# AleoNet/snarkVM

Hardware: AMD Instinct MI355X
Metric: BLS12-377 G1 MSM scalar-point pairs/sec (+ Fr NTT elements/sec in ntt_*) (higher is better)
Workload: dtype u32 limbs (29-bit radix) modular integer arithmetic, Fq 377-bit / Fr 253-bit; 1 GPU; G1 Pippenger MSM 2^24 (BASELINE.json configs[1]), bases (i+1)G registered in HBM, uniform scalars in HBM; independent instance per GPU; scalars=uniform, lg_ntt=24, window_bits=auto, base_tables=12, table_bits=22, pipelined_batch=True

## Files before the change

### snarkvm_amd/csrc/msm.hip.h

```cpp
#pragma once
#include <stdlib.h>

#include <type_traits>

#include "ec.hip.h"
#include "ffl.hip.h"
#include "ffl2.hip.h"
#include "hex2.hip.h"
#include "tuning.hip.h"

namespace sv {

struct msm_plan_t {
    size_t n;
    int c;
    int W;
    int J;
    int Wd;
    uint32_t nb;
    uint32_t nbt;
    uint32_t chunk;
    uint32_t nchunks;
    uint32_t S, S2;
    uint32_t L;
    int rounds;
    uint32_t bias[10];
};

static inline int msm_pick_c(size_t n) {
    if (n > ((size_t)1 << 17)) return 16;
    int lg = 0;
    while (((size_t)1 << lg) < n) lg++;
    int c = lg - 4;
    if (c < 2) c = 2;
    if (c > 11) c = 11;
    return c;
}
static constexpr int MSM_C_MAX = 23;
static constexpr int MSM_BIAS_BITS = 288;
static inline msm_plan_t msm_make_plan(size_t n, int c_override = 0, int tables = 1, int table_bits = 0) {
    msm_plan_t p;
    p.n = n;
    p.J = tables < 1 ? 1 : tables;
    if (p.J == 1) {
        p.c = c_override ? c_override : msm_pick_c(n);
        if (p.c > 16) p.c = 16;
        p.W = (254 + p.c - 1) / p.c;
    } else {
        const int part = table_bits > 0 ? table_bits : 256 / p.J;
        if (c_override) {
            p.c = c_override;
            if (p.c > part) p.c = part;
            while (part % p.c) p.c--;
            if (p.c > 16 && p.c != part) {
                p.c = 16;
                while (part % p.c) p.c--;
            }
            if (p.c < 2) p.c = part <= 16 ? part : 2;
        } else if (part <= 16) {
            p.c = n >= 4096 ? 16 : 8;
            if (p.c > part) p.c = part;
            while (part % p.c) p.c--;
            if (p.c < 2) p.c = part;
        } else {
            double best = 0;
            p.c = 0;
            for (int d = 2; d <= part && d <= MSM_C_MAX; d++) {
                if (part % d || (d > 16 && d != part)) continue;
                const double cost = (double)p.J * (part / d) * (double)n + (double)(part / d) * (double)((size_t)1 << (d - 1)) * 8.0;
                if (p.c == 0 || cost < best) {
                    best = cost;
                    p.c = d;
                }
            }
            if (p.c == 0) p.c = 1;
        }
        p.W = part / p.c;
    }
    p.Wd = p.W * p.J;
    p.nb = 1u << (p.c - 1);
    p.nbt = (uint32_t)p.W * p.nb;
    p.chunk = (1u << 18) / (uint32_t)p.J;
    p.chunk &= ~7u;
    if (p.chunk > n) p.chunk = (uint32_t)(n ? n : 1);
    p.nchunks = (uint32_t)((n + p.chunk - 1) / p.chunk);
    const int env_S = tuning().seg, env_S2 = tuning().seg2, env_L = tuning().fold_l;
    {
        const size_t E = (size_t)p.Wd * n;
        const size_t smax = E >= ((size_t)1 << 27) ? 128 : 64, round = (size_t)1 << 16;
        const size_t k = (E + smax * round - 1) / (smax * round);
        const size_t sfill = k ? (E + k * round - 1) / (k * round) : 4;
        p.S = (uint32_t)(sfill < 4 ? 4 : sfill);
    }
    if (env_S > 0) p.S = env_S;
    p.S2 = env_S2 > 1 ? env_S2 : 16;
    p.L = env_L > 0 ? (uint32_t)env_L : 8;
    if (p.L > p.nb) p.L = p.nb;
    while (p.nb % p.L) p.L--;
    p.rounds = 0;
    size_t m = ((size_t)p.J * n + p.S - 1) / p.S;
    while (m > 1) {
        m = (m + p.S2 - 1) / p.S2;
        p.rounds++;
    }
    for (int i = 0; i < 10; i++) p.bias[i] = 0;
    for (int w = 0; w < p.Wd; w++) {
        int bit = p.c - 1 + p.c * w;
        if (bit >= MSM_BIAS_BITS) break;
        p.bias[bit / 32] |= 1u << (bit % 32);
    }
    return p;
}

static constexpr int SCAN_TILE = 2048;
static __global__ void scan_tile_kernel(const uint32_t* in, uint32_t* out, uint32_t* block_sums, size_t n) {
    __shared__ uint32_t sh[256];
    const size_t base = (size_t)blockIdx.x * SCAN_TILE + (size_t)threadIdx.x * 8;
    uint32_t v[8], s = 0;
#pragma unroll
    for (int i = 0; i < 8; i++) {
        v[i] = (base + i < n) ? in[base + i] : 0u;
        s += v[i];
    }
    sh[threadIdx.x] = s;
    __syncthreads();
    for (int off = 1; off < 256; off <<= 1) {
        uint32_t t = (threadIdx.x >= (unsigned)off) ? sh[threadIdx.x - off] : 0u;
        __syncthreads();
        sh[threadIdx.x] += t;
        __syncthreads();
    }
    uint32_t run = sh[threadIdx.x] - s;
#pragma unroll
    for (int i = 0; i < 8; i++) {
        if (base + i < n) out[base + i] = run;
        run += v[i];
    }
    if (threadIdx.x == 255 && block_sums) block_sums[blockIdx.x] = sh[255];
}
static __global__ void scan_add_kernel(uint32_t* out, const uint32_t* block_offsets, size_t n) {
    const size_t base = (size_t)blockIdx.x * SCAN_TILE + (size_t)threadIdx.x * 8;
    const uint32_t add = block_offsets[blockIdx.x];
#pragma unroll
    for (int i = 0; i < 8; i++)
        if (base + i < n) out[base + i] += add;
}
static inline size_t scan_tmp_elems(size_t n) {
// ... 765 lines not shown
```

### snarkvm_amd/csrc/msm_sort.hip.h

```cpp
#pragma once
#include "ffl.hip.h"
#include "ffl2.hip.h"
#include "ffl2p.hip.h"
#include "msm.hip.h"

namespace sv {

static constexpr int SORT_TILE = 8192;
static constexpr int SORT_THREADS = 256;

struct msm_inst_t {
    const uint4* scalars;
    uint32_t n;
    uint32_t n0;
    uint32_t off0, off1;
    uint32_t pstart;
    uint32_t ptiles;
};
struct msm_radix_params_t {
    size_t n;
    int c, W, J;
    int HB, LB;
    uint32_t nb;
    uint32_t tiles_per_row;
    uint32_t TPW;
    const msm_inst_t* inst = nullptr;
    uint32_t ninst = 0;
    uint32_t vstride = 0, vn0 = 0, vr0 = 0, vr1 = 0;
    uint32_t xcd = 0;
};
__device__ __forceinline__ uint32_t xcd_tile(uint32_t b, uint32_t T) {
    const uint32_t q = T >> 3, r = T & 7u, x = b & 7u;
    return (x < r ? x * (q + 1) : r * (q + 1) + (x - r) * q) + (b >> 3);
}
struct l1_tile_t {
    uint32_t w, tw, TPW, j;
    size_t cbase;
    size_t row;
    size_t lo, hi;
    uint32_t inst_idx;
};
__device__ __forceinline__ l1_tile_t l1_decode_tile(const msm_radix_params_t& p, uint32_t g) {
    l1_tile_t t;
    const uint32_t B1 = 1u << p.HB;
    if (!p.inst) {
        t.w = g / p.TPW;
        t.tw = g - t.w * p.TPW;
        t.TPW = p.TPW;
        t.j = t.tw / p.tiles_per_row;
        const uint32_t tt = t.tw - t.j * p.tiles_per_row;
        t.cbase = (size_t)t.w * B1 * p.TPW;
        t.row = (size_t)(t.j * p.W + t.w) * p.n;
        t.lo = (size_t)tt * SORT_TILE;
        t.hi = (t.lo + SORT_TILE < p.n) ? t.lo + SORT_TILE : p.n;
        t.inst_idx = 0;
        return t;
    }
// ... 690 lines not shown
__global__ void __launch_bounds__(256, 1) msm_accumulate_lazy_kernel(const g1_aff_mem_t* __restrict__ bases, const uint32_t* __restrict__ sorted,
                                                              const uint32_t* __restrict__ boff, const uint32_t* __restrict__ start,
                                                              g1_lazy_partial_t* __restrict__ partial, uint32_t nbt, uint32_t S, uint32_t debug_idx_mask) {
    const uint32_t t = blockIdx.x * blockDim.x + threadIdx.x;
    const uint32_t total = boff[nbt];
    const uint64_t lo64 = (uint64_t)t * S;
    if (lo64 >= total) return;
    const uint32_t lo = (uint32_t)lo64;
    const uint32_t hi = (total - lo < S) ? total : lo + S;
    uint32_t k = find_bucket(boff, nbt, lo);
    uint32_t kend = boff[k + 1];
    uint32_t kend2 = boff[k + 2 <= nbt ? k + 2 : nbt];
    uint32_t start_k = start[k];
    uint32_t part_off = t - boff[k] / S;
    xyzz_lazy_t acc = xyzz_lazy_t::infinity();
    auto slot_of = [&](uint32_t e) -> const g1_lazy_slot_t* { return (const g1_lazy_slot_t*)&bases[(e & 0x7fffffffu) & debug_idx_mask]; };
    uint32_t e_cur = sorted[lo];
    uint32_t e_n1 = lo + 1 < hi ? sorted[lo + 1] : 0u;
    g1_lazy_slot_t raw_next = *slot_of(e_cur);
    for (uint32_t pos = lo;; pos++) {
        const bool end = pos >= hi;
        if (end || pos >= kend) {
            acc.store_raw(&partial[start_k + part_off]);
            if (end) break;
            part_off = 0;
            acc.inf = true;
            k++;
            kend = kend2;
            while (pos >= kend) {
                k++;
                kend = boff[k + 1];
            }
            kend2 = boff[k + 2 <= nbt ? k + 2 : nbt];
            start_k = start[k];
        }
        const uint32_t e = e_cur;
        const g1_lazy_slot_t raw = raw_next;
        if (pos + 1 < hi) raw_next = *slot_of(e_n1);
        e_cur = e_n1;
        if (pos + 2 < hi) e_n1 = sorted[pos + 2];
        if (raw.w[26]) continue;
        const bool neg = (e >> 31) != 0;
        fql_t px, py;
        raw.coords(px, py);
        if (!acc.madd(px, py, neg)) {
            xyzz_lazy_t tmp = acc;
            const fql_t tx = px, ty = py;
            lazy_exceptional_add(&tmp, &tx, &ty, neg);
            acc = tmp;
        }
    }
}

static __global__ void __launch_bounds__(256) g2_pair_partials_to_exact_kernel(const g2_pair_partial_t* __restrict__ raw, xyzz_mem_t<fq2_t>* __restrict__ partial,
                                                                        const uint32_t* __restrict__ start, uint32_t nbt) {
    const uint32_t g = blockIdx.x * blockDim.x + threadIdx.x;
    const uint32_t i = g >> 3, k = g & 7;
    if (i >= start[nbt]) return;
    const uint4* q = (const uint4*)&raw[i].w[16 * k];
    uint32_t t[16];
#pragma unroll
    for (int j = 0; j < 4; j++) {
        const uint4 u = q[j];
        t[4 * j] = u.x, t[4 * j + 1] = u.y, t[4 * j + 2] = u.z, t[4 * j + 3] = u.w;
    }
    fql_t c;
#pragma unroll
    for (int j = 0; j < 13; j++) c.v[j] = (int32_t)t[j];
    c.to_exact().store(&((fq_mem_t*)&partial[i])[k]);
}
template <bool PREFETCH>
__global__ void __launch_bounds__(256, 2) msm_accumulate_pair2_kernel(const aff_mem_t<fq2_t>* __restrict__ bases, const uint32_t* __restrict__ sorted,
                                                               const uint32_t* __restrict__ boff, const uint32_t* __restrict__ start,
                                                               g2_pair_partial_t* __restrict__ partial, uint32_t nbt, uint32_t S, uint32_t debug_idx_mask) {
    const uint32_t gt = blockIdx.x * blockDim.x + threadIdx.x;
    const uint32_t t = gt >> 1;
    const int comp = (int)(gt & 1u);
    const uint32_t total = boff[nbt];
    const uint64_t lo64 = (uint64_t)t * S;
    if (lo64 >= total) return;
    const uint32_t lo = (uint32_t)lo64;
    const uint32_t hi = (total - lo < S) ? total : lo + S;
    uint32_t k = find_bucket(boff, nbt, lo);
    uint32_t kend = boff[k + 1];
    uint32_t start_k = start[k];
    uint32_t part_off = t - boff[k] / S;
    fq2p::xyzz_pair_t<fq2p::xp_dev> acc;
    acc.inf = true;
    auto slot_of = [&](uint32_t e) -> const g2_lazy_slot_t* { return (const g2_lazy_slot_t*)&bases[(e & 0x7fffffffu) & debug_idx_mask]; };
    for (uint32_t pos = lo;; pos++) {
        const bool end = pos >= hi;
        if (end || pos >= kend) {
            uint4* q = (uint4*)&partial[start_k + part_off].w[16 * comp];
            if (acc.inf) {
#pragma unroll
                for (int c4 = 0; c4 < 4; c4++)
#pragma unroll
                    for (int j = 0; j < 4; j++) q[8 * c4 + j] = make_uint4(0, 0, 0, 0);
            } else {
                const fql_t* cs[4] = {&acc.x[0], &acc.y[0], &acc.zz[0], &acc.zzz[0]};
#pragma unroll
                for (int c4 = 0; c4 < 4; c4++) {
                    const int32_t* v = cs[c4]->v;
                    q[8 * c4 + 0] = make_uint4((uint32_t)v[0], (uint32_t)v[1], (uint32_t)v[2], (uint32_t)v[3]);
                    q[8 * c4 + 1] = make_uint4((uint32_t)v[4], (uint32_t)v[5], (uint32_t)v[6], (uint32_t)v[7]);
                    q[8 * c4 + 2] = make_uint4((uint32_t)v[8], (uint32_t)v[9], (uint32_t)v[10], (uint32_t)v[11]);
// ... 23 lines not shown
```

### snarkvm_amd/csrc/runtime.hip.h

```cpp
#pragma once
#include <hip/hip_runtime.h>
#include <stdint.h>
#include <stdio.h>
#include <stdlib.h>
#include <string.h>
#include <time.h>

#include <atomic>
#include <chrono>
#include <condition_variable>
#include <deque>
#include <functional>
#include <exception>
#include <memory>
#include <mutex>
#include <stdexcept>
#include <string>
#include <thread>
#include <type_traits>
#include <utility>
#include <vector>

#include "../../include/snarkvm_hip.h"
#include "ec.hip.h"
// ... 53 lines not shown
        size_t want = bytes + bytes / 8 + 256;
        alloc_timer_t timer(0, want);
        if (p) sv_defer_free(p);
        p = nullptr;
        cap = 0;
        if (hipMalloc(&p, want) != hipSuccess) {
            (void)hipGetLastError();
            p = nullptr;
            sv_drain_frees();
            const hipError_t e = hipMalloc(&p, want);
            if (e != hipSuccess) {
                (void)hipGetLastError();
                p = nullptr;
                throw hip_failure{e, "hipMalloc", __LINE__};
            }
        }
        cap = want;
    }
    template <class T>
    T* as() const {
        return (T*)p;
    }
};
struct pinned_buf {
    void* p = nullptr;
    size_t cap = 0;
    void ensure(size_t bytes) {
        if (bytes <= cap) return;
        size_t want = bytes + bytes / 8 + 4096;
        alloc_timer_t timer(2, want);
        if (p) HIP_TRY(hipHostFree(p));
        p = nullptr;
        cap = 0;
        HIP_TRY(hipHostMalloc(&p, want, hipHostMallocDefault));
        cap = want;
    }
    template <class T>
    T* as() const {
        return (T*)p;
    }
};

struct phase_rec {
    const char* name;
    hipEvent_t e0, e1;
    double ms;
};
struct device_t;

struct lane_t {
    device_t* dev = nullptr;
    int index = 0;
    hipStream_t stream = nullptr;
    dev_buf scalars, digits, counts, offsets, scan_tmp, sorted, boff, cnt_a, cnt_b, start_a, start_b, part_a, part_b, part_raw, planes;
    dev_buf rv1, rl1, rcounts2, roff2, rbinstart, rntiles, rtstart, rbsize;
    dev_buf rv2, rl2, rmid_size, rmid_boff;
    dev_buf fold_sums;
    dev_buf tail_flags;
    dev_buf sink_acc;
    dev_buf fchunk;
    dev_buf bases_tmp, scalars_tmp, gen_pts, gen_prod;
    dev_buf ntt_data, ntt_scratch, ntt_acc, ntt_alt;
    dev_buf serde_status;
    dev_buf poly[5];
    pinned_buf pin, pin2;
    hipStream_t alt = nullptr;
    hipEvent_t ev[4] = {};
    std::vector<void*> tw_leases;
    bool in_scope = false;
    struct deferred_out_t {
        void* dst;
        size_t off, bytes;
    };
    std::vector<deferred_out_t> deferred;
    size_t deferred_bytes = 0;
    size_t pin_used = 0;
    std::vector<hipEvent_t> scope_events;
    size_t scope_events_used = 0;
    hipEvent_t scope_event() {
        if (scope_events_used == scope_events.size()) {
            hipEvent_t e;
            HIP_TRY(hipEventCreateWithFlags(&e, hipEventDisableTiming));
            scope_events.push_back(e);
        }
        return scope_events[scope_events_used++];
    }
    std::vector<phase_rec> phases;
    std::vector<hipEvent_t> event_pool;
    size_t events_used = 0;

    hipEvent_t new_event() {
        if (events_used == event_pool.size()) {
            hipEvent_t e;
            HIP_TRY(hipEventCreate(&e));
            event_pool.push_back(e);
        }
        return event_pool[events_used++];
    }
    inline ntt_ctx_t ntt_ctx(hipStream_t st = nullptr);
    inline void begin_call();
    inline void phase_begin(const char* name);
    inline void phase_end();
    inline void phase_host(const char* name, double ms);
    inline void end_call();
    void sync_or_defer() {
        if (!in_scope) HIP_TRY(hipStreamSynchronize(stream));
    }
// ... 142 lines not shown
        if (e != hipSuccess || ndev == 0) throw hip_failure{e == hipSuccess ? hipErrorNoDevice : e, "hipGetDeviceCount (no MI355X visible)", __LINE__};
        std::vector<int> ids = want;
        if (ids.empty()) {
            if (const char* env = getenv("SNARKVM_HIP_DEVICES")) {
                for (const char* p = env; *p;) {
                    char* end = nullptr;
                    long v = strtol(p, &end, 10);
                    if (end == p) break;
                    ids.push_back((int)v);
                    p = (*end == ',') ? end + 1 : end;
                }
            }
        }
        if (ids.empty())
            for (int d = 0; d < ndev; d++) ids.push_back(d);
        for (int id : ids)
            if (id < 0 || id >= ndev) throw hip_failure{hipErrorInvalidDevice, "device index out of range (snarkvm_hip_set_devices / SNARKVM_HIP_DEVICES)", __LINE__};
        for (size_t i = 0; i < ids.size(); i++) {
            devs.emplace_back(new device_t());
            devs.back()->logical = (int)i;
            devs.back()->physical = ids[i];
        }
        configured = true;
    }
    int ndev() {
        configure();
        return (int)devs.size();
    }
    int device_of(const void* ptr) {
        configure();
        hipPointerAttribute_t at;
        if (!ptr || hipPointerGetAttributes(&at, ptr) != hipSuccess) {
            (void)hipGetLastError();
            return -1;
        }
        std::vector<int> match;
        for (auto& d : devs)
            if (d->physical == at.device) match.push_back(d->logical);
        if (match.empty()) return -1;
        return match[rr.fetch_add(1) % match.size()];
    }
};
extern runtime_t g_rt;

static void tu_kernel_attributes(int logical) {
    static std::mutex mu;
    static std::vector<char> done;
    std::lock_guard<std::mutex> lk(mu);
    if ((int)done.size() <= logical) done.resize(logical + 1, 0);
    if (done[logical]) return;
    HIP_TRY(hipFuncSetAttribute((const void*)scan_one_block_kernel, hipFuncAttributeMaxDynamicSharedMemorySize, (int)(SCAN_ONE_MAX * 4)));
#ifdef SV_TU_G1
    HIP_TRY(hipFuncSetAttribute((const void*)msm_accumulate_lazy_kernel<true>, hipFuncAttributeMaxDynamicSharedMemorySize, 128 * 1024));
#endif
#ifdef SV_TU_NTT
    HIP_TRY(hipFuncSetAttribute((const void*)ntt_pass_kernel_v2<false, ntt_arith_u>, hipFuncAttributeMaxDynamicSharedMemorySize, 96 * 1024));
    HIP_TRY(hipFuncSetAttribute((const void*)ntt_pass_kernel_v2<true, ntt_arith_u>, hipFuncAttributeMaxDynamicSharedMemorySize, 96 * 1024));
    HIP_TRY(hipFuncSetAttribute((const void*)ntt_pass_kernel_v2<true, ntt_arith_u, ntt_load_bounded>, hipFuncAttributeMaxDynamicSharedMemorySize, 96 * 1024));
    HIP_TRY(hipFuncSetAttribute((const void*)ntt_pass_kernel_v2<false, ntt_arith_u, ntt_load_product>, hipFuncAttributeMaxDynamicSharedMemorySize, 96 * 1024));
#endif
    done[logical] = 1;
}

static constexpr int SCOPE_AUX_MAX = 7;
struct scope_pending_t {
    hipEvent_t done;
    std::function<void()> finish;
    const void* tag;
};
struct thread_scope_t {
    lane_t* lane = nullptr;
    int prev_device = -1;
    unsigned flags = 0;
    lane_t* aux[SCOPE_AUX_MAX] = {};
    int naux = 0;
    unsigned aux_rr = 0;
    bool aux_exhausted = false;
    std::vector<scope_pending_t> pending;
    thread_scope_t() = default;
    thread_scope_t(const thread_scope_t&) = default;
    thread_scope_t& operator=(const thread_scope_t&) = default;
    ~thread_scope_t();
};
extern thread_local thread_scope_t g_tl_scope;
static thread_scope_t& tl_scope() { return g_tl_scope; }
static void scope_flush() {
    thread_scope_t& sc = tl_scope();
    if (!sc.lane) return;
    std::exception_ptr err;
    for (scope_pending_t& p : sc.pending) {
        try {
            HIP_TRY(hipEventSynchronize(p.done));
            p.finish();
        } catch (...) {
            if (!err) err = std::current_exception();
        }
    }
    sc.pending.clear();
    try {
        sc.lane->flush_scope();
        for (int i = 0; i < sc.naux; i++) HIP_TRY(hipStreamSynchronize(sc.aux[i]->stream));
    } catch (...) {
        if (!err) err = std::current_exception();
    }
    sc.lane->pin_used = 0;
    sc.lane->scope_events_used = 0;
// ... 410 lines not shown
    const char* cur = "";
    void begin(const char* name) {
        cur = name;
        if (trace >= 2) fprintf(stderr, "[snarkvm_hip] msm n=%zu: %s ...\n", n, name);
        if (profile) c.phase_begin(name);
    }
    void end() {
        if (profile) c.phase_end();
        if (trace >= 2) {
            const hipError_t e = hipStreamSynchronize(c.stream);
            fprintf(stderr, "[snarkvm_hip] msm n=%zu: %s done (%s)\n", n, cur, hipGetErrorString(e));
        }
    }
};
template <class T>
static void msm_reduce_and_tail(lane_t& c, const msm_plan_t& pl, const msm_tail_geom_t& tg, uint32_t nwin, uint32_t nbt, int rounds, size_t T0_max, size_t T1_max,
                                const msm_bucket_sink_t* sink, msm_pending_t& pd, void* host_planes, msm_phases_t& ph) {
    hipStream_t st = c.stream;
    ph.begin("msm_reduce_partials");
    uint32_t *cnt_in = c.cnt_a.as<uint32_t>(), *cnt_out = c.cnt_b.as<uint32_t>();
    uint32_t *start_in = c.start_a.as<uint32_t>(), *start_out = c.start_b.as<uint32_t>();
    xyzz_mem_t<T> *pin = c.part_a.as<xyzz_mem_t<T>>(), *pout = c.part_b.as<xyzz_mem_t<T>>();
    size_t T_in_max = T0_max;
    for (int r = 0; r < rounds; r++) {
        size_t T_out_max = T_in_max / pl.S2 + nbt + 1;
        if (T_out_max > T1_max) T_out_max = T1_max;
        hipLaunchKernelGGL(msm_alloc_kernel, dim3((nbt + 1 + 255) / 256), dim3(256), 0, st, cnt_in, cnt_out, nbt, pl.S2);
        exclusive_scan_u32(st, cnt_out, start_out, (size_t)nbt + 1, c.scan_tmp.as<uint32_t>());
        hipLaunchKernelGGL((msm_reduce_kernel<T>), dim3((unsigned)((T_out_max + 255) / 256)), dim3(256), 0, st, pin, start_in, cnt_in, start_out, pout, nbt,
                           pl.S2);
        std::swap(cnt_in, cnt_out);
        std::swap(start_in, start_out);
        std::swap(pin, pout);
        T_in_max = T_out_max;
    }
    ph.end();
    if (sink) {
        ph.begin("msm_bucket_merge");
        if (sink->after) HIP_TRY(hipStreamWaitEvent(st, sink->after, 0));
        hipLaunchKernelGGL((msm_bucket_merge_kernel<T>), dim3((nbt + 255) / 256), dim3(256), 0, st, (const xyzz_mem_t<T>*)pin, (const uint32_t*)start_in,
                           (const uint32_t*)cnt_in, (xyzz_mem_t<T>*)sink->acc, nbt, sink->L, sink->slot);
        if (sink->done) HIP_TRY(hipEventRecord(sink->done, st));
        ph.end();
        HIP_TRY(hipGetLastError());
        pd.nplanes = 0;
        return;
    }
    ph.begin("msm_bucket_reduce");
    msm_tail_launch<T>(c, pl, tg, nwin, nbt, pin, start_in, cnt_in, pd, host_planes);
    ph.end();
}
template <class F>
static void msm_launch_accumulate(lane_t& c, const msm_plan_t& pl, const aff_mem_t<F>* vbase, uint32_t* boffp, uint32_t nbt, size_t nthreads, bool one_wave,
                                  bool ltail) {
    hipStream_t st = c.stream;
#ifdef SV_BENCH
    static const uint32_t dbg_mask = getenv("SNARKVM_HIP_DEBUG_IDX_MASK") ? (uint32_t)strtoul(getenv("SNARKVM_HIP_DEBUG_IDX_MASK"), nullptr, 0) : 0xffffffffu;
#else
    constexpr uint32_t dbg_mask = 0xffffffffu;
#endif
    const size_t tmax = nthreads + nbt + 1;
    if constexpr (sizeof(F) == sizeof(fq_t)) {
        if (msm_lazy_on<F>()) {
            if (!ltail) c.part_raw.ensure(tmax * sizeof(g1_lazy_partial_t));
            g1_lazy_partial_t* raw_out = ltail ? c.part_a.as<g1_lazy_partial_t>() : c.part_raw.as<g1_lazy_partial_t>();
            hipLaunchKernelGGL((msm_accumulate_lazy_kernel<true>), dim3((unsigned)((nthreads + 255) / 256)), dim3(256), one_wave || tuning().acc_one_wg ? msm_acc_lds() : 0, st,
                               vbase, c.sorted.as<uint32_t>(), boffp, c.start_a.as<uint32_t>(), raw_out, nbt, pl.S, dbg_mask);
            if (!ltail)
                hipLaunchKernelGGL(g1_partials_to_exact_kernel, dim3((unsigned)((tmax + 255) / 256)), dim3(256), 0, st, (const g1_lazy_partial_t*)raw_out,
                                   c.part_a.as<g1_xyzz_mem_t>(), (const uint32_t*)c.start_a.as<uint32_t>(), nbt);
            return;
        }
    } else {
#ifndef SV_NO_G2
        if (msm_lazy_on<F>()) {
            c.part_raw.ensure(tmax * sizeof(g2_pair_partial_t));
            hipLaunchKernelGGL((msm_accumulate_pair2_kernel<false>), dim3((unsigned)((2 * nthreads + 255) / 256)), dim3(256), 0, st, vbase, c.sorted.as<uint32_t>(),
                               boffp, c.start_a.as<uint32_t>(), c.part_raw.as<g2_pair_partial_t>(), nbt, pl.S, dbg_mask);
            hipLaunchKernelGGL(g2_pair_partials_to_exact_kernel, dim3((unsigned)((8 * tmax + 255) / 256)), dim3(256), 0, st,
                               (const g2_pair_partial_t*)c.part_raw.as<g2_pair_partial_t>(), c.part_a.as<xyzz_mem_t<fq2_t>>(),
                               (const uint32_t*)c.start_a.as<uint32_t>(), nbt);
            return;
        }
#endif
    }
    if (one_wave)
        hipLaunchKernelGGL((msm_accumulate_seg_kernel<F, 1, true>), dim3((unsigned)((nthreads + 255) / 256)), dim3(256), 0, st, vbase, c.sorted.as<uint32_t>(), boffp,
                           c.start_a.as<uint32_t>(), c.part_a.as<xyzz_mem_t<F>>(), nbt, pl.S, dbg_mask);
    else
        hipLaunchKernelGGL((msm_accumulate_seg_kernel<F, 1, false>), dim3((unsigned)((nthreads + 255) / 256)), dim3(256), 0, st, vbase, c.sorted.as<uint32_t>(), boffp,
                           c.start_a.as<uint32_t>(), c.part_a.as<xyzz_mem_t<F>>(), nbt, pl.S, dbg_mask);
}
template <class F>
static size_t msm_plane_bytes() {
    return (size_t)MSM_MAX_POS * msm_point_bytes<F>();
}
template <class F>
struct msm_job_t {
    const aff_mem_t<F>* bases = nullptr;
    const aff_mem_t<F>* bases1 = nullptr;
    size_t n0 = 0;
    int tables = 1;
    size_t table_stride = 0;
    int table_bits = 0;
    const uint4* scalars = nullptr;
    size_t n = 0;
    int scalars_montgomery = 0;
    int window_bits = 0;
    void* host_planes = nullptr;
    bool profile = true;
    const msm_multi_t* multi = nullptr;
    const msm_bucket_sink_t* sink = nullptr;
    hipEvent_t scalars_read = nullptr;
};
template <class F>
struct msm_layout_t {
    msm_plan_t pl;
    bool wide;
    bool fused;
    bool ltail;
    bool single_round, prefetch_ok;
    uint32_t nwin, nbt;
    size_t E_max, T0_max, T1_max;
    const aff_mem_t<F>* vbase;
    msm_tail_geom_t tg;
    msm_radix_params_t rp;
    msm_digit_params_t dp;
    int LBL;
    uint32_t B1, nbins, nseg_last;
    size_t ncounts1, tiles1, tiles2_max;
};
template <class F>
static msm_layout_t<F> msm_layout(lane_t& c, const msm_job_t<F>& j, msm_pending_t& pd) {
    const msm_multi_t* mu = j.multi;
    const size_t n = j.n;
    size_t n0 = j.bases1 ? j.n0 : n;
    if (n0 > n) n0 = n;
    msm_layout_t<F> L{};
    if (n >= ((size_t)1 << 31)) throw hip_failure{hipErrorInvalidValue, "msm: npoints must be < 2^31", __LINE__};
    const msm_plan_t pl = L.pl = msm_make_plan(n, mu ? j.table_bits : j.window_bits, j.tables, j.table_bits);
    L.wide = pl.c > 16;
    if (mu && (L.wide || pl.W != 1 || pl.c < 12 || (size_t)pl.J * mu->hn >= ((size_t)1 << 31) || n != mu->npad || n % SORT_TILE))
        throw hip_failure{hipErrorInvalidValue, "msm: geometry not eligible for a fused multi-instance run", __LINE__};
    if ((size_t)pl.Wd * n >= ((size_t)1 << 32)) throw hip_failure{hipErrorInvalidValue, "msm: windows * npoints must be < 2^32", __LINE__};
    if ((size_t)pl.J * n >= ((size_t)1 << 31)) throw hip_failure{hipErrorInvalidValue, "msm: tables * npoints must be < 2^31", __LINE__};
    const aff_mem_t<F>* vb1 = j.bases1 ? j.bases1 : j.bases;
    L.vbase = mu ? j.bases : (vb1 < j.bases ? vb1 : j.bases);
    if (!mu) {
        const size_t top0 = (size_t)(j.bases - L.vbase) + n0, top1 = (size_t)(vb1 - L.vbase) + (n - n0);
        if ((size_t)(pl.J - 1) * j.table_stride + (top0 > top1 ? top0 : top1) >= ((size_t)1 << 31))
            throw hip_failure{hipErrorInvalidValue, "msm: base slots must be addressable in 31 bits (tables * registered points < 2^31)", __LINE__};
    }
    const size_t E_max = L.E_max = (size_t)pl.Wd * n;
    const uint32_t nwin = L.nwin = mu ? mu->K : (uint32_t)pl.W;
    const uint32_t nbt = L.nbt = nwin * pl.nb;

    c.scan_tmp.ensure((scan_tmp_elems((size_t)nbt + 1)) * 4);
    c.boff.ensure(((size_t)nbt + 2) * 4);
    c.cnt_a.ensure(((size_t)nbt + 1) * 4);
    c.cnt_b.ensure(((size_t)nbt + 1) * 4);
    c.start_a.ensure(((size_t)nbt + 1) * 4);
    c.start_b.ensure(((size_t)nbt + 1) * 4);
    const size_t slack = (size_t)nbt / 32 + 64;
    L.T0_max = E_max / pl.S + nbt + 1 + slack;
    L.T1_max = L.T0_max / pl.S2 + nbt + 1 + slack;
    pd.lazy = L.ltail = msm_lazy_tail_on<F>();
    c.part_a.ensure(L.T0_max * msm_partial_bytes<F>());
    c.part_b.ensure(L.T1_max * msm_partial_bytes<F>());
    L.tg = msm_tail_geometry(pl, nwin, pd, mu ? (int)mu->K : 0);
    if (mu && (size_t)pd.nplanes > mu->plane_capacity) throw hip_failure{hipErrorInvalidValue, "msm: plane staging of the fused group too small", __LINE__};
    if (j.sink && (mu || j.sink->nbt != nbt)) throw hip_failure{hipErrorInvalidValue, "msm: bucket sink does not match the plan", __LINE__};
    c.planes.ensure((size_t)pd.nplanes * msm_partial_bytes<F>());

    L.fused = !mu && L.wide && tuning().fused && pl.c <= 22 && pl.Wd <= FUSED_MAX_ROWS;
    memcpy(L.dp.bias, pl.bias, sizeof L.dp.bias);
    L.dp.c = pl.c;
    L.dp.W = pl.Wd;
    L.dp.n = n;
    L.dp.montgomery = j.scalars_montgomery;
    L.single_round = mu || (size_t)pl.Wd * n <= ((size_t)1 << 22);
    L.prefetch_ok = (size_t)pl.Wd * n <= ((size_t)1 << 22);

    msm_radix_params_t& rp = L.rp;
    rp.n = n;
    rp.c = pl.c;
    rp.W = pl.W;
    rp.J = pl.J;
    if (mu) {
        rp.inst = mu->d_inst;
        rp.ninst = mu->K;
        rp.vstride = (uint32_t)mu->hn;
    } else {
        rp.vn0 = (uint32_t)n0;
        rp.vr0 = (uint32_t)(j.bases - L.vbase);
        rp.vr1 = (uint32_t)(vb1 - L.vbase);
        rp.vstride = (uint32_t)j.table_stride;
    }
    const int K = pl.c - 1;
    L.LBL = K < 7 ? K : 7;
    rp.LB = L.wide ? 14 : L.LBL;
    rp.HB = K - rp.LB;
    rp.nb = pl.nb;
    rp.xcd = (uint32_t)tuning().xcd;
    rp.tiles_per_row = L.fused ? (uint32_t)((n + FUSED_TILE - 1) / FUSED_TILE) : (uint32_t)((n + SORT_TILE - 1) / SORT_TILE);
    rp.TPW = (uint32_t)pl.J * rp.tiles_per_row;
    L.B1 = 1u << rp.HB;
    L.nbins = nwin * L.B1;
    L.ncounts1 = (size_t)(mu ? L.B1 : L.nbins) * rp.TPW;
    L.tiles1 = (size_t)(mu ? 1 : pl.W) * rp.TPW;
    L.nseg_last = L.wide ? L.nbins << 7 : L.nbins;
    L.tiles2_max = E_max / SORT_TILE + L.nseg_last + 1;
    return L;
}
template <class F>
static void msm_stage_digits(lane_t& c, const msm_layout_t<F>& L, const msm_job_t<F>& j, msm_phases_t& ph) {
    hipStream_t st = c.stream;
    ph.begin("msm_digits");
    c.digits.ensure(L.E_max * (L.wide ? sizeof(uint32_t) : sizeof(uint16_t)));
    size_t blocks = (j.n + 255) / 256;
    if (j.multi) {
        hipLaunchKernelGGL(msm_digits_multi_kernel, dim3((unsigned)blocks), dim3(256), 0, st, j.multi->d_inst, j.multi->K, c.digits.as<uint16_t>(), L.dp);
    } else {
        if (blocks > 256 * 16) blocks = 256 * 16;
        if (L.wide)
            hipLaunchKernelGGL((msm_digits_kernel<uint32_t>), dim3((unsigned)blocks), dim3(256), 0, st, j.scalars, c.digits.as<uint32_t>(), L.dp);
        else
            hipLaunchKernelGGL((msm_digits_kernel<uint16_t>), dim3((unsigned)blocks), dim3(256), 0, st, j.scalars, c.digits.as<uint16_t>(), L.dp);
    }
    ph.end();
    if (j.scalars_read) HIP_TRY(hipEventRecord(j.scalars_read, st));
}
template <class Fn>
static void msm_fused_width(int c, Fn&& fn) {
    switch (c) {
// ... 101 lines not shown
    const uint32_t* seg_start = c.rbinstart.as<uint32_t>();
    uint32_t nseg = L.nbins;
    const uint32_t* v_in = c.rv1.as<uint32_t>();
    if (L.wide) {
        ph.begin("msm_sort_level2");
        const uint32_t ngroups = nseg << 7;
        const size_t tmax = E_max / SORT_TILE + nseg + 1;
        c.rv2.ensure(E_max * 4);
        c.rl2.ensure(E_max);
        c.rmid_size.ensure(((size_t)ngroups + 3) * 4);
        c.rmid_boff.ensure(((size_t)ngroups + 3) * 4);
        c.scan_tmp.ensure(scan_tmp_elems((size_t)ngroups + 2) * 4);
        uint32_t* msize = c.rmid_size.as<uint32_t>();
        uint32_t* mboff = c.rmid_boff.as<uint32_t>();
        msm_tile_segments(c, seg_start, nseg);
        hipLaunchKernelGGL((radix_hist2_kernel<uint16_t>), dim3((unsigned)tmax), dim3(SORT_THREADS), 0, st, c.rl1.as<uint16_t>(), seg_start,
                           c.rtstart.as<uint32_t>(), c.rcounts2.as<uint32_t>(), nseg, 7, 7);
        HIP_TRY(hipMemsetAsync(msize + ngroups + 1, 0, 4, st));
        msm_colscan(c, msize, nseg, 7, msize + ngroups + 1);
        exclusive_scan_u32(st, msize, mboff, (size_t)ngroups + 1, c.scan_tmp.as<uint32_t>());
        hipLaunchKernelGGL((radix_scatter2_kernel<uint16_t, uint8_t>), dim3((unsigned)tmax), dim3(SORT_THREADS), 0, st, v_in, c.rl1.as<uint16_t>(),
                           seg_start, c.rtstart.as<uint32_t>(), c.rcounts2.as<uint32_t>(), c.roff2.as<uint32_t>(), mboff, c.rv2.as<uint32_t>(),
                           c.rl2.as<uint8_t>(), nseg, 7, 7, (uint32_t)tuning().xcd);
        ph.end();
        seg_start = mboff;
        nseg = ngroups;
        v_in = c.rv2.as<uint32_t>();
    }
    ph.begin(L.wide ? "msm_sort_level3" : "msm_sort_level2");
    msm_tile_segments(c, seg_start, nseg);
    const uint8_t* rem_last = L.wide ? c.rl2.as<uint8_t>() : c.rl1.as<uint8_t>();
    hipLaunchKernelGGL((radix_hist2_kernel<uint8_t>), dim3((unsigned)L.tiles2_max), dim3(SORT_THREADS), 0, st, rem_last, seg_start,
                       c.rtstart.as<uint32_t>(), c.rcounts2.as<uint32_t>(), nseg, L.LBL, 0);
    HIP_TRY(hipMemsetAsync(d_max, 0, 4, st));
    msm_colscan(c, bsize, nseg, L.LBL, d_max);
    exclusive_scan_u32(st, bsize, boffp, (size_t)nbt + 1, c.scan_tmp.as<uint32_t>());
    hipLaunchKernelGGL((radix_scatter2_kernel<uint8_t, uint8_t>), dim3((unsigned)L.tiles2_max), dim3(SORT_THREADS), 0, st, v_in, rem_last, seg_start,
                       c.rtstart.as<uint32_t>(), c.rcounts2.as<uint32_t>(), c.roff2.as<uint32_t>(), boffp, c.sorted.as<uint32_t>(),
                       (uint8_t*)nullptr, nseg, L.LBL, 0, (uint32_t)tuning().xcd);
    ph.end();
}
template <class F>
static int msm_stage_accumulate(lane_t& c, const msm_layout_t<F>& L, const msm_job_t<F>& j, msm_phases_t& ph) {
    hipStream_t st = c.stream;
    const msm_multi_t* mu = j.multi;
    const uint32_t nbt = L.nbt;
    uint32_t* boffp = c.boff.as<uint32_t>();
    int rounds = 0;
    ph.begin("msm_accumulate");
    const int env_rounds = tuning().reduce_rounds;
    if (!L.single_round) rounds = env_rounds < 0 ? 0 : (env_rounds > 8 ? 8 : env_rounds);
    if (mu && tuning().fuse_reduce > 0) rounds = tuning().fuse_reduce > 4 ? 4 : tuning().fuse_reduce;
    if (mu && tuning().fuse_reduce < 0) rounds = mu->K >= 8 ? 1 : 0;
    hipLaunchKernelGGL(msm_alloc_seg_kernel, dim3((nbt + 1 + 255) / 256), dim3(256), 0, st, boffp, c.cnt_a.as<uint32_t>(), nbt, L.pl.S);
    exclusive_scan_u32(st, c.cnt_a.as<uint32_t>(), c.start_a.as<uint32_t>(), (size_t)nbt + 1, c.scan_tmp.as<uint32_t>());
    msm_launch_accumulate<F>(c, L.pl, L.vbase, boffp, nbt, (L.E_max + L.pl.S - 1) / L.pl.S, L.single_round && L.prefetch_ok, L.ltail);
    ph.end();
    return rounds;
}
template <class T>
struct msm_field_tag {
    using type = T;
};
template <class F, class Fn>
static void msm_on_tail_field(bool lazy, Fn&& fn) {
    if constexpr (sizeof(F) == sizeof(fq_t)) {
        if (lazy) return fn(msm_field_tag<fqz_t>{});
    }
    fn(msm_field_tag<F>{});
}
template <class F>
static msm_pending_t msm_run(lane_t& c, const msm_job_t<F>& j) {
    msm_pending_t pd;
    pd.planes = j.host_planes;
    if (j.n == 0) return pd;
    msm_phases_t ph{c, j.profile, msm_trace_level(), j.n};
    const msm_layout_t<F> L = msm_layout(c, j, pd);
    if (!L.fused) msm_stage_digits(c, L, j, ph);
    msm_stage_level1(c, L, j, ph);
    msm_stage_sort_rest(c, L, ph);
    const int rounds = msm_stage_accumulate(c, L, j, ph);
    msm_on_tail_field<F>(L.ltail, [&](auto t) {
        msm_reduce_and_tail<typename decltype(t)::type>(c, L.pl, L.tg, L.nwin, L.nbt, rounds, L.T0_max, L.T1_max, j.sink, pd, j.host_planes, ph);
    });
    return pd;
}
template <class F>
static msm_pending_t msm_tail_from_sink(lane_t& c, const msm_job_t<F>& j, const msm_bucket_sink_t& sink) {
    msm_pending_t pd;
    pd.planes = j.host_planes;
    const msm_plan_t pl = msm_make_plan(j.n, j.window_bits, j.tables, j.table_bits);
    const uint32_t nwin = (uint32_t)pl.W, nbt = nwin * pl.nb;
    if (nbt != sink.nbt) throw hip_failure{hipErrorInvalidValue, "msm: bucket sink does not match the plan", __LINE__};
    const msm_tail_geom_t tg = msm_tail_geometry(pl, nwin, pd, 0);
    c.start_a.ensure(((size_t)nbt + 1) * 4);
    c.cnt_a.ensure(((size_t)nbt + 1) * 4);
    hipLaunchKernelGGL(msm_sink_lists_kernel, dim3((nbt + 1 + 255) / 256), dim3(256), 0, c.stream, c.start_a.as<uint32_t>(), c.cnt_a.as<uint32_t>(), nbt, sink.L);
    pd.lazy = msm_lazy_tail_on<F>();
    c.phase_begin("msm_bucket_reduce");
    msm_on_tail_field<F>(pd.lazy, [&](auto t) {
        using T = typename decltype(t)::type;
        msm_tail_launch<T>(c, pl, tg, nwin, nbt, (const xyzz_mem_t<T>*)sink.acc, c.start_a.as<uint32_t>(), c.cnt_a.as<uint32_t>(), pd, j.host_planes);
    });
    c.phase_end();
    return pd;
}
// ... 840 lines not shown
```

### snarkvm_amd/csrc/tuning.hip.h

```cpp
#pragma once
#include <stdio.h>
#include <stdlib.h>
#include <string.h>

namespace sv {

struct tuning_t {
    int lazy = 1, lazy2 = 1, fused = 1;
    long acc_lds = 96 * 1024;
    int acc_one_wg = 0, reduce_rounds = 1, fuse_batch = 1, fuse_max_k = 64, fuse_reduce = -1, coalesce = 1, coalesce_us = 40, lanes = 0;
    int msm_chunk_lg = 20, scalar_chunk_lg = 22, taper = 1, ring_lanes = 3, seg = 0, seg2 = 0, fold_l = 0, scan1 = 1;
    int ntt_min_tiles = 256, ntt_full_tw = 1, ntt_fold = 1, ntt_batch = 1;
    int xcd = 1, fold_threads2 = 128, coalesce_slots = 2, ramp = 3, scalar_geo = 4, lazy_tail = 1, horner2 = 1, hex2 = 1, group_quad = 1, tail_quads = 13, fold_small2 = 256, fold_mid = 128;

    bool set(const char* key, long v) {
#define SV_TUNE_KEY(name)                  \
    if (!strcmp(key, #name)) {             \
        name = (decltype(name))v;          \
        return true;                       \
    }
        SV_TUNE_KEY(lazy) SV_TUNE_KEY(lazy2) SV_TUNE_KEY(fused) SV_TUNE_KEY(acc_lds)
        SV_TUNE_KEY(acc_one_wg) SV_TUNE_KEY(reduce_rounds) SV_TUNE_KEY(fuse_batch) SV_TUNE_KEY(fuse_max_k) SV_TUNE_KEY(fuse_reduce) SV_TUNE_KEY(coalesce)
        SV_TUNE_KEY(coalesce_us) SV_TUNE_KEY(lanes) SV_TUNE_KEY(msm_chunk_lg) SV_TUNE_KEY(scalar_chunk_lg) SV_TUNE_KEY(taper) SV_TUNE_KEY(ring_lanes) SV_TUNE_KEY(seg) SV_TUNE_KEY(seg2)
        SV_TUNE_KEY(fold_l) SV_TUNE_KEY(scan1) SV_TUNE_KEY(ntt_min_tiles) SV_TUNE_KEY(ntt_full_tw) SV_TUNE_KEY(ntt_fold)
        SV_TUNE_KEY(ntt_batch) SV_TUNE_KEY(xcd) SV_TUNE_KEY(fold_threads2) SV_TUNE_KEY(coalesce_slots) SV_TUNE_KEY(ramp) SV_TUNE_KEY(scalar_geo) SV_TUNE_KEY(lazy_tail) SV_TUNE_KEY(horner2) SV_TUNE_KEY(hex2) SV_TUNE_KEY(group_quad) SV_TUNE_KEY(tail_quads) SV_TUNE_KEY(fold_small2) SV_TUNE_KEY(fold_mid)
#undef SV_TUNE_KEY
        return false;
    }
    void parse(const char* s) {
        while (s && *s) {
            while (*s == ',' || *s == ' ') s++;
            const char* eq = strchr(s, '=');
            const char* end = strchr(s, ',');
            if (!end) end = s + strlen(s);
            if (!*s) break;
            char key[32] = {0};
            if (!eq || eq > end || (size_t)(eq - s) >= sizeof key) {
                fprintf(stderr, "[snarkvm_hip] SNARKVM_HIP_TUNING: malformed item at \"%s\" (ignored)\n", s);
            } else {
                memcpy(key, s, (size_t)(eq - s));
                char* num_end = nullptr;
                const long v = strtol(eq + 1, &num_end, 0);
                if (num_end == eq + 1 || !set(key, v)) fprintf(stderr, "[snarkvm_hip] SNARKVM_HIP_TUNING: unknown key or bad value \"%s\" (ignored)\n", key);
            }
            s = end;
        }
    }
    void clamp() {
        auto fix = [](const char* key, auto& v, long lo, long hi) {
            if ((long)v < lo || (long)v > hi) {
                const long was = (long)v;
                v = (decltype(v + 0))((long)v < lo ? lo : hi);
                fprintf(stderr, "[snarkvm_hip] SNARKVM_HIP_TUNING: %s=%ld is out of range [%ld, %ld]; using %ld\n", key, was, lo, hi, (long)v);
            }
        };
        fix("coalesce_slots", coalesce_slots, 1, 8);
        fix("coalesce_us", coalesce_us, 0, 100000);
        fix("fuse_max_k", fuse_max_k, 2, 256);
        fix("fuse_reduce", fuse_reduce, -1, 4);
        fix("reduce_rounds", reduce_rounds, 0, 8);
        fix("lanes", lanes, 0, 8);
        fix("ring_lanes", ring_lanes, 2, 8);
        fix("ntt_min_tiles", ntt_min_tiles, 1, 1 << 20);
        fix("acc_lds", acc_lds, 0, 160 * 1024);
        fix("msm_chunk_lg", msm_chunk_lg, 16, 30);
        fix("scalar_chunk_lg", scalar_chunk_lg, 18, 30);
        fix("ramp", ramp, 0, 6);
        fix("scalar_geo", scalar_geo, 0, 16);
        fix("seg", seg, 0, 4096);
        fix("seg2", seg2, 0, 256);
        fix("fold_l", fold_l, 0, 64);
    }
};
inline const tuning_t& tuning() {
    static const tuning_t t = [] {
        tuning_t v;
        v.parse(getenv("SNARKVM_HIP_TUNING"));
        v.clamp();
        return v;
    }();
    return t;
}

}
```

Measured before the change: 575.5 million pairs/s.

## Add length-binned bucket accumulation with capped, balanced per-thread chunks

Adds a binned path for large lazy G1 MSMs. Each bucket is split into evenly sized chunks of at most `cap` points, with `cap` set to about 1.5× the mean bucket load. Within each 4096-item tile, the work items are counting-sorted by chunk length, so threads in a wavefront run loops of similar length and finish close together. This aims to cut divergence and tail idle time in the accumulate kernel, replacing fixed-S segmenting. The cost is two extra kernels, an extra items buffer and uint4 indirection loads per thread.

```diff
diff --git a/snarkvm_amd/csrc/msm.hip.h b/snarkvm_amd/csrc/msm.hip.h
--- a/snarkvm_amd/csrc/msm.hip.h
+++ b/snarkvm_amd/csrc/msm.hip.h
@@ -22,6 +22,7 @@
     uint32_t chunk;
     uint32_t nchunks;
     uint32_t S, S2;
+    uint32_t cap;
     uint32_t L;
     int rounds;
     uint32_t bias[10];
@@ -93,6 +94,12 @@
         p.S = (uint32_t)(sfill < 4 ? 4 : sfill);
     }
     if (env_S > 0) p.S = env_S;
+    {
+        const size_t mean = (size_t)p.Wd * n / p.nbt, want = (mean * 3 / 2) & ~(size_t)31;
+        p.cap = (uint32_t)(want < 64 ? 64 : want > 255 ? 255 : want);
+        const int env_cap = tuning().acc_cap;
+        if (env_cap > 0) p.cap = (uint32_t)env_cap;
+    }
     p.S2 = env_S2 > 1 ? env_S2 : 16;
     p.L = env_L > 0 ? (uint32_t)env_L : 8;
     if (p.L > p.nb) p.L = p.nb;
diff --git a/snarkvm_amd/csrc/msm_chunks.hip.h b/snarkvm_amd/csrc/msm_chunks.hip.h
--- /dev/null
+++ b/snarkvm_amd/csrc/msm_chunks.hip.h
@@ -0,0 +1,20 @@
+#pragma once
+#include <hip/hip_runtime.h>
+#include <stdint.h>
+
+#ifndef SV_HD
+#define SV_HD __host__ __device__ __forceinline__
+#endif
+
+namespace sv {
+
+struct acc_chunk_t {
+    uint32_t off, len;
+};
+SV_HD uint32_t acc_chunk_count(uint32_t len, uint32_t cap) { return len / cap + (len % cap ? 1u : 0u); }
+SV_HD acc_chunk_t acc_chunk(uint32_t len, uint32_t cap, uint32_t j) {
+    const uint32_t nch = acc_chunk_count(len, cap), q = len / nch, r = len % nch;
+    return {j * q + (j < r ? j : r), q + (j < r ? 1u : 0u)};
+}
+
+}
diff --git a/snarkvm_amd/csrc/msm_sort.hip.h b/snarkvm_amd/csrc/msm_sort.hip.h
--- a/snarkvm_amd/csrc/msm_sort.hip.h
+++ b/snarkvm_amd/csrc/msm_sort.hip.h
@@ -3,6 +3,7 @@
 #include "ffl2.hip.h"
 #include "ffl2p.hip.h"
 #include "msm.hip.h"
+#include "msm_chunks.hip.h"
 
 namespace sv {
 
@@ -799,6 +800,113 @@
     }
 }
 
+static __global__ void msm_alloc_bins_kernel(const uint32_t* __restrict__ boff, uint32_t* __restrict__ cnt, uint32_t nbt, uint32_t cap) {
+    const uint32_t k = blockIdx.x * blockDim.x + threadIdx.x;
+    if (k > nbt) return;
+    cnt[k] = k < nbt ? acc_chunk_count(boff[k + 1] - boff[k], cap) : 0u;
+}
+static constexpr int BIN_TILE = 4096;
+static constexpr int BIN_THREADS = 1024;
+static constexpr int BIN_CAP_MAX = 255;
+static __global__ void __launch_bounds__(BIN_THREADS) msm_bin_items_kernel(const uint32_t* __restrict__ boff, const uint32_t* __restrict__ start,
+                                                                          uint4* __restrict__ items, uint32_t nbt, uint32_t cap) {
+    __shared__ uint32_t hist[BIN_CAP_MAX + 1], first[BIN_CAP_MAX + 1];
+    const uint32_t total = start[nbt];
+    const uint32_t t0 = blockIdx.x * BIN_TILE;
+    if (t0 >= total) return;
+    if (threadIdx.x <= BIN_CAP_MAX) hist[threadIdx.x] = 0;
+    __syncthreads();
+    constexpr int PER = BIN_TILE / BIN_THREADS;
+    uint4 rec[PER];
+    uint32_t rank[PER];
+#pragma unroll
+    for (int q = 0; q < PER; q++) {
+        const uint32_t slot = t0 + q * BIN_THREADS + threadIdx.x;
+        rec[q] = make_uint4(0, 0, 0, 0);
+        rank[q] = 0;
+        if (slot < total) {
+            const uint32_t k = find_bucket(start, nbt, slot);
+            const uint32_t lo = boff[k];
+            const acc_chunk_t ch = acc_chunk(boff[k + 1] - lo, cap, slot - start[k]);
+            rec[q] = make_uint4(lo + ch.off, ch.len, slot, k);
+            rank[q] = atomicAdd(&hist[ch.len], 1u);
+        }
+    }
+    __syncthreads();
+    if (threadIdx.x <= BIN_CAP_MAX) {
+        uint32_t s = 0;
+        for (uint32_t l = threadIdx.x + 1; l <= BIN_CAP_MAX; l++) s += hist[l];
+        first[threadIdx.x] = s;
+    }
+    __syncthreads();
+    const bool full = total - t0 >= BIN_TILE;
+#pragma unroll
+    for (int q = 0; q < PER; q++)
+        if (rec[q].y) {
+            const uint32_t r = first[rec[q].y] + rank[q];
+            uint32_t wg = r >> 8;
+            if (full && wg >= 8) wg = 23 - wg;
+            items[t0 + (wg << 8) + (r & 255u)] = rec[q];
+        }
+}
+template <bool PREFETCH>
+__global__ void __launch_bounds__(256, 1) msm_accumulate_binned_kernel(const g1_aff_mem_t* __restrict__ bases, const uint32_t* __restrict__ sorted,
+                                                                const uint4* __restrict__ items, const uint32_t* __restrict__ start,
+                                                                g1_lazy_partial_t* __restrict__ partial, uint32_t nbt, uint32_t debug_idx_mask) {
+    const uint32_t t = blockIdx.x * blockDim.x + threadIdx.x;
+    const bool valid = t < start[nbt];
+    const uint4 it = valid ? items[t] : make_uint4(0, 0, 0, 0);
+    const uint32_t* ent = sorted + it.x;
+    const uint32_t len = it.y;
+    uint32_t wmax = len;
+#pragma unroll
+    for (int o = 32; o; o >>= 1) {
+        const uint32_t other = (uint32_t)__shfl_xor((int)wmax, o);
+        wmax = other > wmax ? other : wmax;
+    }
+    wmax = (uint32_t)__builtin_amdgcn_readfirstlane((int)wmax);
+    if (wmax == 0) return;
+    xyzz_lazy_t acc = xyzz_lazy_t::infinity();
+    auto slot_of = [&](uint32_t e) -> const g1_lazy_slot_t* { return (const g1_lazy_slot_t*)&bases[(e & 0x7fffffffu) & debug_idx_mask]; };
+    const uint32_t last = len ? len - 1 : 0u;
+    uint32_t e_cur = ent[0];
+    uint32_t e_n1 = ent[last < 1 ? last : 1];
+    g1_lazy_slot_t raw_next = *slot_of(e_cur);
+    auto take = [&](uint32_t i, uint32_t& e, g1_lazy_slot_t& raw) {
+        e = e_cur;
+        raw = raw_next;
+        raw_next = *slot_of(e_n1);
+        e_cur = e_n1;
+        e_n1 = ent[i + 2 < last ? i + 2 : last];
+    };
+    {
+        uint32_t e;
+        g1_lazy_slot_t raw;
+        take(0, e, raw);
+        if (len && !raw.w[26]) {
+            fql_t px, py;
+            raw.coords(px, py);
+            acc.madd(px, py, (e >> 31) != 0);
+        }
+    }
+    for (uint32_t i = 1; i < wmax; i++) {
+        uint32_t e;
+        g1_lazy_slot_t raw;
+        take(i, e, raw);
+        if (i >= len || raw.w[26]) continue;
+        const bool neg = (e >> 31) != 0;
+        fql_t px, py;
+        raw.coords(px, py);
+        if (!acc.madd(px, py, neg)) {
+            xyzz_lazy_t tmp = acc;
+            const fql_t tx = px, ty = py;
+            lazy_exceptional_add(&tmp, &tx, &ty, neg);
+            acc = tmp;
+        }
+    }
+    if (valid) acc.store_raw(&partial[it.z]);
+}
+
 static __global__ void __launch_bounds__(256) g2_pair_partials_to_exact_kernel(const g2_pair_partial_t* __restrict__ raw, xyzz_mem_t<fq2_t>* __restrict__ partial,
                                                                         const uint32_t* __restrict__ start, uint32_t nbt) {
     const uint32_t g = blockIdx.x * blockDim.x + threadIdx.x;
diff --git a/snarkvm_amd/csrc/runtime.hip.h b/snarkvm_amd/csrc/runtime.hip.h
--- a/snarkvm_amd/csrc/runtime.hip.h
+++ b/snarkvm_amd/csrc/runtime.hip.h
@@ -129,7 +129,7 @@
     device_t* dev = nullptr;
     int index = 0;
     hipStream_t stream = nullptr;
-    dev_buf scalars, digits, counts, offsets, scan_tmp, sorted, boff, cnt_a, cnt_b, start_a, start_b, part_a, part_b, part_raw, planes;
+    dev_buf scalars, digits, counts, offsets, scan_tmp, sorted, boff, cnt_a, cnt_b, start_a, start_b, part_a, part_b, part_raw, acc_items, planes;
     dev_buf rv1, rl1, rcounts2, roff2, rbinstart, rntiles, rtstart, rbsize;
     dev_buf rv2, rl2, rmid_size, rmid_boff;
     dev_buf fold_sums;
@@ -378,6 +378,7 @@
     HIP_TRY(hipFuncSetAttribute((const void*)scan_one_block_kernel, hipFuncAttributeMaxDynamicSharedMemorySize, (int)(SCAN_ONE_MAX * 4)));
 #ifdef SV_TU_G1
     HIP_TRY(hipFuncSetAttribute((const void*)msm_accumulate_lazy_kernel<true>, hipFuncAttributeMaxDynamicSharedMemorySize, 128 * 1024));
+    HIP_TRY(hipFuncSetAttribute((const void*)msm_accumulate_binned_kernel<true>, hipFuncAttributeMaxDynamicSharedMemorySize, 128 * 1024));
 #endif
 #ifdef SV_TU_NTT
     HIP_TRY(hipFuncSetAttribute((const void*)ntt_pass_kernel_v2<false, ntt_arith_u>, hipFuncAttributeMaxDynamicSharedMemorySize, 96 * 1024));
@@ -894,20 +895,24 @@
 }
 template <class F>
 static void msm_launch_accumulate(lane_t& c, const msm_plan_t& pl, const aff_mem_t<F>* vbase, uint32_t* boffp, uint32_t nbt, size_t nthreads, bool one_wave,
-                                  bool ltail) {
+                                  bool ltail, bool binned = false) {
     hipStream_t st = c.stream;
 #ifdef SV_BENCH
     static const uint32_t dbg_mask = getenv("SNARKVM_HIP_DEBUG_IDX_MASK") ? (uint32_t)strtoul(getenv("SNARKVM_HIP_DEBUG_IDX_MASK"), nullptr, 0) : 0xffffffffu;
 #else
     constexpr uint32_t dbg_mask = 0xffffffffu;
 #endif
-    const size_t tmax = nthreads + nbt + 1;
+    const size_t tmax = binned ? nthreads : nthreads + nbt + 1;
     if constexpr (sizeof(F) == sizeof(fq_t)) {
         if (msm_lazy_on<F>()) {
             if (!ltail) c.part_raw.ensure(tmax * sizeof(g1_lazy_partial_t));
             g1_lazy_partial_t* raw_out = ltail ? c.part_a.as<g1_lazy_partial_t>() : c.part_raw.as<g1_lazy_partial_t>();
-            hipLaunchKernelGGL((msm_accumulate_lazy_kernel<true>), dim3((unsigned)((nthreads + 255) / 256)), dim3(256), one_wave || tuning().acc_one_wg ? msm_acc_lds() : 0, st,
-                               vbase, c.sorted.as<uint32_t>(), boffp, c.start_a.as<uint32_t>(), raw_out, nbt, pl.S, dbg_mask);
+            if (binned)
+                hipLaunchKernelGGL((msm_accumulate_binned_kernel<true>), dim3((unsigned)((nthreads + 255) / 256)), dim3(256), one_wave || tuning().acc_one_wg ? msm_acc_lds() : 0, st,
+                                   vbase, c.sorted.as<uint32_t>(), (const uint4*)c.acc_items.as<uint4>(), (const uint32_t*)c.start_a.as<uint32_t>(), raw_out, nbt, dbg_mask);
+            else
+                hipLaunchKernelGGL((msm_accumulate_lazy_kernel<true>), dim3((unsigned)((nthreads + 255) / 256)), dim3(256), one_wave || tuning().acc_one_wg ? msm_acc_lds() : 0, st,
+                                   vbase, c.sorted.as<uint32_t>(), boffp, c.start_a.as<uint32_t>(), raw_out, nbt, pl.S, dbg_mask);
             if (!ltail)
                 hipLaunchKernelGGL(g1_partials_to_exact_kernel, dim3((unsigned)((tmax + 255) / 256)), dim3(256), 0, st, (const g1_lazy_partial_t*)raw_out,
                                    c.part_a.as<g1_xyzz_mem_t>(), (const uint32_t*)c.start_a.as<uint32_t>(), nbt);
@@ -962,6 +967,7 @@
     bool fused;
     bool ltail;
     bool single_round, prefetch_ok;
+    bool binned;
     uint32_t nwin, nbt;
     size_t E_max, T0_max, T1_max;
     const aff_mem_t<F>* vbase;
@@ -1003,8 +1009,15 @@
     c.cnt_b.ensure(((size_t)nbt + 1) * 4);
     c.start_a.ensure(((size_t)nbt + 1) * 4);
     c.start_b.ensure(((size_t)nbt + 1) * 4);
+    L.single_round = mu || (size_t)pl.Wd * n <= ((size_t)1 << 22);
+    L.prefetch_ok = (size_t)pl.Wd * n <= ((size_t)1 << 22);
+    L.binned = false;
+    if constexpr (sizeof(F) == sizeof(fq_t))
+        L.binned = msm_lazy_on<F>() && !mu && (tuning().acc_bins == 2 || (tuning().acc_bins == 1 && !L.single_round && nbt >= (1u << 19)));
     const size_t slack = (size_t)nbt / 32 + 64;
-    L.T0_max = E_max / pl.S + nbt + 1 + slack;
+    const uint32_t per_sum = L.binned && pl.cap < pl.S ? pl.cap : pl.S;
+    L.T0_max = E_max / per_sum + nbt + 1 + slack;
+    if (L.binned) c.acc_items.ensure(L.T0_max * sizeof(uint4));
     L.T1_max = L.T0_max / pl.S2 + nbt + 1 + slack;
     pd.lazy = L.ltail = msm_lazy_tail_on<F>();
     c.part_a.ensure(L.T0_max * msm_partial_bytes<F>());
@@ -1020,8 +1033,6 @@
     L.dp.W = pl.Wd;
     L.dp.n = n;
     L.dp.montgomery = j.scalars_montgomery;
-    L.single_round = mu || (size_t)pl.Wd * n <= ((size_t)1 << 22);
-    L.prefetch_ok = (size_t)pl.Wd * n <= ((size_t)1 << 22);
 
     msm_radix_params_t& rp = L.rp;
     rp.n = n;
@@ -1229,6 +1240,15 @@
     if (!L.single_round) rounds = env_rounds < 0 ? 0 : (env_rounds > 8 ? 8 : env_rounds);
     if (mu && tuning().fuse_reduce > 0) rounds = tuning().fuse_reduce > 4 ? 4 : tuning().fuse_reduce;
     if (mu && tuning().fuse_reduce < 0) rounds = mu->K >= 8 ? 1 : 0;
+    if (L.binned) {
+        hipLaunchKernelGGL(msm_alloc_bins_kernel, dim3((nbt + 1 + 255) / 256), dim3(256), 0, st, boffp, c.cnt_a.as<uint32_t>(), nbt, L.pl.cap);
+        exclusive_scan_u32(st, c.cnt_a.as<uint32_t>(), c.start_a.as<uint32_t>(), (size_t)nbt + 1, c.scan_tmp.as<uint32_t>());
+        hipLaunchKernelGGL(msm_bin_items_kernel, dim3((unsigned)((L.T0_max + BIN_TILE - 1) / BIN_TILE)), dim3(BIN_THREADS), 0, st, (const uint32_t*)boffp,
+                           (const uint32_t*)c.start_a.as<uint32_t>(), c.acc_items.as<uint4>(), nbt, L.pl.cap);
+        msm_launch_accumulate<F>(c, L.pl, L.vbase, boffp, nbt, L.T0_max, L.single_round && L.prefetch_ok, L.ltail, true);
+        ph.end();
+        return rounds;
+    }
     hipLaunchKernelGGL(msm_alloc_seg_kernel, dim3((nbt + 1 + 255) / 256), dim3(256), 0, st, boffp, c.cnt_a.as<uint32_t>(), nbt, L.pl.S);
     exclusive_scan_u32(st, c.cnt_a.as<uint32_t>(), c.start_a.as<uint32_t>(), (size_t)nbt + 1, c.scan_tmp.as<uint32_t>());
     msm_launch_accumulate<F>(c, L.pl, L.vbase, boffp, nbt, (L.E_max + L.pl.S - 1) / L.pl.S, L.single_round && L.prefetch_ok, L.ltail);
diff --git a/snarkvm_amd/csrc/tuning.hip.h b/snarkvm_amd/csrc/tuning.hip.h
--- a/snarkvm_amd/csrc/tuning.hip.h
+++ b/snarkvm_amd/csrc/tuning.hip.h
@@ -12,6 +12,7 @@
     int msm_chunk_lg = 20, scalar_chunk_lg = 22, taper = 1, ring_lanes = 3, seg = 0, seg2 = 0, fold_l = 0, scan1 = 1;
     int ntt_min_tiles = 256, ntt_full_tw = 1, ntt_fold = 1, ntt_batch = 1;
     int xcd = 1, fold_threads2 = 128, coalesce_slots = 2, ramp = 3, scalar_geo = 4, lazy_tail = 1, horner2 = 1, hex2 = 1, group_quad = 1, tail_quads = 13, fold_small2 = 256, fold_mid = 128;
+    int acc_bins = 1, acc_cap = 0;
 
     bool set(const char* key, long v) {
 #define SV_TUNE_KEY(name)                  \
@@ -24,6 +25,7 @@
         SV_TUNE_KEY(coalesce_us) SV_TUNE_KEY(lanes) SV_TUNE_KEY(msm_chunk_lg) SV_TUNE_KEY(scalar_chunk_lg) SV_TUNE_KEY(taper) SV_TUNE_KEY(ring_lanes) SV_TUNE_KEY(seg) SV_TUNE_KEY(seg2)
         SV_TUNE_KEY(fold_l) SV_TUNE_KEY(scan1) SV_TUNE_KEY(ntt_min_tiles) SV_TUNE_KEY(ntt_full_tw) SV_TUNE_KEY(ntt_fold)
         SV_TUNE_KEY(ntt_batch) SV_TUNE_KEY(xcd) SV_TUNE_KEY(fold_threads2) SV_TUNE_KEY(coalesce_slots) SV_TUNE_KEY(ramp) SV_TUNE_KEY(scalar_geo) SV_TUNE_KEY(lazy_tail) SV_TUNE_KEY(horner2) SV_TUNE_KEY(hex2) SV_TUNE_KEY(group_quad) SV_TUNE_KEY(tail_quads) SV_TUNE_KEY(fold_small2) SV_TUNE_KEY(fold_mid)
+        SV_TUNE_KEY(acc_bins) SV_TUNE_KEY(acc_cap)
 #undef SV_TUNE_KEY
         return false;
     }
@@ -70,6 +72,8 @@
         fix("seg", seg, 0, 4096);
         fix("seg2", seg2, 0, 256);
         fix("fold_l", fold_l, 0, 64);
+        fix("acc_bins", acc_bins, 0, 2);
+        fix("acc_cap", acc_cap, 0, 255);
     }
 };
 inline const tuning_t& tuning() {
```

After: 541.5 million pairs/s. -5.9%, worse.
